# AI-Unicamp/GestureDiffusion

Hardware: AMD Instinct MI355X
Metric: denoised motion frames/sec (1000-step p_sample_loop, B=64, T=196, d=512) (higher is better)
Workload: dtype f32; 1 GPU; BASELINE config 2: MDM_Old (V1 encoder-only topology) J=263 d=512 ff=1024 L=8 H=4, 1000-step p_sample_loop, batch 64/GPU x 196 frames, random weights, in-kernel Philox noise; global_batch=64, frames=196, parallelism=dp1 (independent samples, end-of-loop gather), step=one denoising step (forward + fused sampler update) over the rank's batch

## Files before the change

gesturediffusion_amd/_lib.py:

```python
import ctypes as C
import os

_HERE = os.path.dirname(os.path.abspath(__file__))
LIB_PATH = os.environ.get("GDX_LIBGDX") or os.path.join(_HERE, "csrc", "libgdx.so")

GDX_ARCH_MDM_OLD, GDX_ARCH_MDM = 1, 2
GDX_COND, GDX_UNCOND, GDX_CFG = 0, 1, 2
GDX_SAMPLER_P, GDX_SAMPLER_DDIM = 0, 1
GDX_ROW_PAD = 256

EXPORTS = [
    "gdx_create", "gdx_destroy", "gdx_last_error", "gdx_set_weight", "gdx_weights_ready", "gdx_prepare",
    "gdx_set_condition", "gdx_forward", "gdx_set_keep_taps", "gdx_get_tap", "gdx_sampler_update", "gdx_q_sample",
    "gdx_randn", "gdx_sample_loop", "gdx_bench_ffn_gemm", "gdx_bench_gemm", "gdx_forward_flops", "gdx_profile_begin", "gdx_profile_end", "gdx_bench_attention",
    "gdx_linear_f16", "gdx_linear_f32", "gdx_bench_gemm_f16", "gdx_attention_f16", "gdx_attention_f32", "gdx_plms_update", "gdx_postprocess", "gdx_q_sample_t", "gdx_masked_l2", "gdx_set_graph_replay", "gdx_mfcc",
    "gdx_set_guards", "gdx_check_guards", "gdx_packed_bytes", "gdx_export_packed", "gdx_import_packed", "gdx_set_test_half_dtype",
    "gdx_set_test_gemmh_tile", "gdx_linear_half", "gdx_layernorm", "gdx_local_attention", "gdx_attention_half",
    "gdx_bpd_terms", "gdx_bpd_loop", "gdx_linear_full", "gdx_plms_step", "gdx_plms_loop",
    "gdx_dpm_step", "gdx_dpm_loop", "gdx_dpm_sde_step", "gdx_dpm_sde_loop",
    "gdx_set_guidance_interval", "gdx_forward_samples", "gdx_set_guidance_rescale", "gdx_cfg_rescale",
    "gdx_set_guidance_refresh", "gdx_cfg_delta",
    "gdx_transpose_in", "gdx_transpose_out", "gdx_small_linear", "gdx_gather_rows", "gdx_mfcc_project", "gdx_token0",
]
GDX_BPD_CHUNK = 4096
INT64_MIN, INT64_MAX = -2**63, 2**63 - 1


class GdxError(RuntimeError):
    pass


class Config(C.Structure):
    _fields_ = [(n, C.c_int32) for n in ("arch", "njoints", "latent_dim", "ff_size", "num_layers", "num_heads",
                                         "seed_poses", "mfcc_dim", "cl_head", "window", "compute_dtype")]


class UpdateArgs(C.Structure):
# ... 155 lines not shown
        "gdx_bench_attention": [i32, i32, i32, i32, i32, i32, C.POINTER(C.c_float), vp],
        "gdx_linear_f16": [vp, vp, vp, vp, vp, i32, i32, i32, i32, vp],
        "gdx_linear_f32": [vp, vp, vp, vp, vp, i32, i32, i32, i32, i32, i32, i32, vp],
        "gdx_linear_half": [vp, vp, vp, vp, i32, vp, i32, vp, vp, i32, i32, i32, i32, i32, i32, i32, i32, i32, i32,
                            C.POINTER(i32), vp],
        "gdx_linear_full": [vp, vp, vp, vp, i32, vp, i32, vp, i32, i32, i32, i32, i32, i32, i32, i32, i32, i32, i32,
                            C.POINTER(i32), vp],
        "gdx_layernorm": [vp, vp, vp, vp, vp, vp, i32, i32, i32, i32, i32, i32, vp],
        "gdx_local_attention": [vp, vp, vp, vp, vp, i32, i32, i32, i32, i32, i32, i32, C.POINTER(i32), vp],
        "gdx_transpose_in": [vp, vp, i32, i32, i32, i32, i32, i32, i32, vp],
        "gdx_transpose_out": [vp, vp, i32, i32, i32, i32, i32, vp],
        "gdx_small_linear": [vp, i32, vp, i32, vp, vp, i32, i32, i32, i32, i32, i32, vp],
        "gdx_gather_rows": [vp, vp, vp, i32, i32, i32, i32, vp],
        "gdx_mfcc_project": [vp, vp, i32, vp, vp, vp, i32, i32, i32, i32, i32, i32, i32, i32, vp],
        "gdx_token0": [vp, i32, vp, vp, vp, vp, i32, vp, vp, vp, i32, vp, i32, i32, i32, i32, i32, vp],
        "gdx_set_graph_replay": [vp, i32],
        "gdx_mfcc": [vp, i64, i32, i32, i32, i32, i32, i32, C.c_float, vp, vp, vp, vp, vp, vp, vp, vp, vp],
        "gdx_q_sample_t": [vp, vp, vp, vp, i32, i64, vp, vp],
        "gdx_masked_l2": [vp, vp, vp, vp, i32, i32, i32, vp],
        "gdx_postprocess": [vp, vp, vp, vp, vp, i32, i32, i32, vp],
        "gdx_plms_update": [C.POINTER(PlmsArgs), vp],
        "gdx_plms_step": [C.POINTER(PlmsStepArgs), vp],
        "gdx_plms_loop": [vp, C.POINTER(PlmsLoopArgs), vp],
        "gdx_dpm_step": [C.POINTER(DpmStepArgs), vp],
        "gdx_dpm_loop": [vp, C.POINTER(DpmLoopArgs), vp],
        "gdx_dpm_sde_step": [C.POINTER(DpmSdeStepArgs), vp],
        "gdx_dpm_sde_loop": [vp, C.POINTER(DpmSdeLoopArgs), vp],
        "gdx_attention_f16": [vp, vp, i32, i32, i32, i32, vp],
        "gdx_attention_half": [vp, i32, vp, i32, i32, i32, i32, i32, i32, i32, i32, C.POINTER(i32), vp],
        "gdx_attention_f32": [vp, vp, i32, i32, i32, i32, i32, vp],
# ... 32 lines not shown
```

gesturediffusion_amd/csrc/api.hip:

```cpp
#include "gdx_host.h"

#include <algorithm>
#include <cstdlib>
#include <cstring>
#include <string>
#include <vector>

namespace gdx {

static thread_local std::string g_err;

int fail(const std::string& m) {
    g_err = m;
    return -1;
}

}

using namespace gdx;

static constexpr size_t GUARD_BYTES = 64 * 1024;
static constexpr int GUARD_BYTE = 0xA5;

int gdx::dev_alloc(std::vector<void*>& pool, void** p, size_t bytes) {
// ... 267 lines not shown
    const int d = h->d;
    const bool res32 = !h->f16 || h->stream32;
    if (res32 ? linear(h, in, W, {.bias = W.bias, .R = resid.f, .ldr = d}, Act{h->tmp.f, nullptr}, d, N, d, s)
              : linear(h, in, W, {.bias = W.bias}, Act{nullptr, h->tmp.h}, d, N, d, s))
        return -1;
    for (const Act* o : {out, compact}) {
        if (!o) continue;
        const int cS = o == compact ? h->S : 0;
        if (res32) HIPCHK(HFN(h->bf16, launch_layernorm, h->tmp.f, nullptr, gamma, beta, o->f, o->h, N, d, cS, s));
        else HIPCHK(HFN(h->bf16, launch_layernorm_f16, h->tmp.h, resid.h, gamma, beta, o->h, o->f, N, d, cS, s));
    }
    return 0;
}

static int forward_core(gdx_model* h, const float* x, const float* temb, int tstride, const float* c2t, int mode,
                        float* x0_out, hipStream_t s, const int* state = nullptr, bool tm = false) {
    const int B = h->B, T = h->T, S = h->S, d = h->d, J = h->J;
    const int Beff = mode == GDX_CFG ? 2 * B : B;
    h->forward_samples += Beff;
    const float* seed_emb = mode == GDX_UNCOND ? h->seed_cat + (size_t)B * d : h->seed_cat;
    const int N = Beff * S;
    const Act xa{!h->f16 || h->stream32 || h->keep_taps ? h->xa.f : nullptr, h->xa.h};
    if (!tm && !h->f16) HIPCHK(launch_transpose_in(x, h->xt.f, Beff, B, J, T, h->in_x.kpad, s));
    if (!tm && h->f16) HIPCHK(HFN(h->bf16, launch_transpose_in_f16, x, h->xt.h, Beff, B, J, T, h->in_x.kpad16, s));
    if (h->cfg.arch == GDX_ARCH_MDM_OLD) {
        HIPCHK(HFN(h->bf16, launch_token0, temb, tstride, seed_emb, h->pe, h->xa.f, h->xa.h, nullptr, nullptr, nullptr, state, Beff, B, S, d, s));
        if (linear(h, h->xt, h->in_x, {.R = h->addend, .ldr = d, .rowmap = true}, xa, d, Beff * T, d, s)) return -1;
    } else {
        if (!c2t) return fail("forward_core: V2 needs the W_coa * temb rows");
        const float* c2s = mode == GDX_UNCOND ? h->c2_seed + (size_t)B * d : h->c2_seed;
        HIPCHK(HFN(h->bf16, launch_token0, temb, tstride, seed_emb, nullptr, h->xa.f, h->xa.h, c2t, c2s, h->c2, state, Beff, B, S, d, s));
        if (linear(h, h->xt, h->in_x, {.bias = h->in_x.bias}, h->emb, d, Beff * T, d, s)) return -1;
        const int dt = h->cfg.compute_dtype;
        const bool la16 = local_attention_half(dt, d, h->cfg.cl_head, h->cfg.window);
        const Act xseq = la16 ? Act{nullptr, h->xseq.h} : Act{h->xseq.f, nullptr};
        if (linear(h, h->emb, h->proj_pose, {.R = h->addend, .ldr = d, .V = h->c2, .ldv = d}, xseq, d, Beff * T, d, s)) return -1;
        HIPCHK(launch_local_attention_any(dt, h->xseq.f, h->xseq.h, h->rope_cos, h->rope_sin, la16 ? xa.f : h->xa.f, h->xa.h, Beff, T,
                                          d, h->cfg.cl_head, h->cfg.window, s));
    }
    auto tap = [&](int l) {
        if (h->keep_taps) HIPCHK(hipMemcpyAsync(h->taps[l], h->xa.f, sizeof(float) * (size_t)N * d, hipMemcpyDeviceToDevice, s));
// ... 186 lines not shown
    if (tables_live) return 0;
    h->tmap_host.assign(timestep_map, timestep_map + num_steps);
    HIPCHK(hipMemcpyAsync(h->tmap_dev, h->tmap_host.data(), sizeof(int64_t) * num_steps, hipMemcpyHostToDevice, s));
    float* scratch0 = table + (size_t)h->temb_table_rows * d;
    float* scratch1 = scratch0 + (size_t)h->temb_table_rows * d;
    if (time_embed(h, h->tmap_dev, num_steps, scratch0, scratch1, table, s)) return -1;
    if (h->cfg.arch == GDX_ARCH_MDM) {
        HIPCHK(launch_small_linear(table, d, h->proj_coa.w, h->proj_coa.kpad, nullptr, h->c2t_table, d, num_steps, d, d, 0, s));
        h->c2t_valid = true;
    }
    h->tables_valid = true;
    return 0;
}

static int denoise_step(gdx_model* h, const float* x, int idx, int mode, float* x0_out, hipStream_t s, const int* state = nullptr,
                        bool tm = false) {
    const size_t row = (size_t)idx * h->d;
    const int fm = mode == GDX_CFG_REFRESH ? GDX_CFG : mode == GDX_CFG_REUSE ? GDX_COND : mode;
    return forward_core(h, x, h->temb_table + row, 0, h->c2t_table ? h->c2t_table + row : nullptr, fm, x0_out, s, state, tm);
}

static const float* tape_slice(const float* tape, int k, int k_base, size_t rows, size_t per) {
    return tape ? tape + (ptrdiff_t)(k - k_base) * (ptrdiff_t)(rows * per) : nullptr;
}

static int denoise_guided(gdx_model* h, const CallSeq& q, const float* sc_in, const float* x, int idx, hipStream_t s,
                          const float** x0_uncond, const float** scale, bool second = false) {
    const int m = step_mode(h, q, idx, second);
    return denoise_step(h, x, idx, m, h->x0, s) || guided_operands(h, m, sc_in, s, x0_uncond, scale) ? -1 : 0;
}

extern "C" int gdx_bpd_loop(gdx_handle_t h, const gdx_bpd_loop_args_t* a, void* stream) {
    if (!h) return fail("gdx_bpd_loop: null handle");
    if (!a) return fail("gdx_bpd_loop: null argument");
// ... 192 lines not shown
    const bool refreshes = h->guide_every > 1 && any_guided;
    if (!((uintptr_t)a->noise_tape & 15) && !a->inpaint_mask && !a->n_dump && !h->graph_replay && !h->keep_taps && h->T % 4 == 0 &&
        !rescales && !refreshes) {
        static const bool mirror_always = [] { const char* e = getenv("GDX_TM_MIRROR"); return e && !strcmp(e, "always"); }();
        const int Beff = any_guided ? 2 * B : B;
        const int ldx = h->f16 ? h->in_x.kpad16 : h->in_x.kpad;
        HIPCHK(launch_transpose_in(a->x, h->xt.f, Beff, B, h->J, h->T, ldx, s));
        if (h->f16) HIPCHK(HFN(h->bf16, launch_transpose_in_f16, a->x, h->xt.h, Beff, B, h->J, h->T, ldx, s));
        gdx::UpdateTmDev u;
        memset(&u, 0, sizeof(u));
        u.kind = a->kind; u.B = B; u.J = h->J; u.T = h->T; u.ldx = ldx; u.ldo = h->ldo;
        u.coef = a->coef; u.xt = h->xt.f; u.x0t = h->x0t;
        u.const_noise = a->const_noise; u.seed = a->philox_seed; u.sample_offset = a->sample_offset;
        u.clip = a->clip_denoised;
        u.xt16 = h->xt.h; u.half_dtype = h->cfg.compute_dtype;
        int k = a->k_base;
        for (int idx = a->first_index; idx >= last_idx; --idx, ++k) {
            const int m = mode_at(idx);
            if (denoise_step(h, nullptr, idx, m, nullptr, s, nullptr, true)) return -1;
            u.scale = m == GDX_CFG ? a->scale : nullptr;
            u.mirror = any_guided && m != GDX_CFG && (mirror_always || (idx > last_idx && mode_at(idx - 1) == GDX_CFG));
            u.step_index = idx; u.rng_step = (uint32_t)(k + 1);
            u.out_pose = idx == last_idx ? a->x : nullptr;
            u.noise = tape_slice(a->noise_tape, k, a->k_base, tape_rows, per);
            if (gdx_sampler_update_tm_(u, stream)) return -1;
        }
        return 0;
    }
    const bool want_graph = h->graph_replay && !h->prof && !h->keep_taps && !a->n_dump && a->first_index - last_idx >= 8 && uniform && !refreshes;
    int idx = a->first_index, k = a->k_base;
    if (want_graph) {
        if (eager_step(idx, k)) return -1;
        --idx; ++k;
        bool ok = true;
// ... 150 lines not shown
```

gesturediffusion_amd/csrc/gdx_internal.h:

```cpp
#pragma once
#include <hip/hip_runtime.h>
#include <stdint.h>

#include "../../include/gdx.h"

#ifdef GDX_BF16
#define GDX_HNS_BEGIN namespace b16 {
#define GDX_HNS_NAME b16
#else
#define GDX_HNS_BEGIN inline namespace h16 {
#define GDX_HNS_NAME h16
#endif
#define GDX_HNS_END }

namespace gdx {

#ifdef GDX_BF16
typedef __bf16 half_t;
#else
typedef _Float16 half_t;
#endif

constexpr int ROW_PAD = GDX_ROW_PAD;

// ... 120 lines not shown
struct UpdateTmDev {
    int kind, B, J, T, ldx, ldo;
    const float* coef; int step_index;
    float* xt;
    const float* x0t;
    const float* scale;
    int const_noise;
    uint64_t seed, sample_offset;
    uint32_t rng_step;
    int clip;
    float* out_pose;
    void* xt16;
    int half_dtype;
    const float* noise;
    int mirror;
};

}

int gdx_sampler_update_state_(const gdx_update_args_t* a, const int* state, long noise_stride, void* stream);
int gdx_sampler_update_tm_(const gdx::UpdateTmDev& d, void* stream);
int gdx_bpd_xt_(const float* x0, const float* coef, int idx, int batch, long per_sample, uint64_t seed, uint64_t sample_offset,
                uint32_t step, float* z_out, float* xt_out, void* stream);
extern "C" int gdx_set_error_(const char* msg);
```

gesturediffusion_amd/csrc/misc.hip:

```cpp
#include "gdx_internal.h"
#include "gdx_device.h"

namespace gdx {
GDX_HNS_BEGIN

__device__ __forceinline__ float wave_sum(float v) {
#pragma unroll
    for (int o = 32; o > 0; o >>= 1) v += __shfl_xor(v, o);
    return v;
}

template <int VPL>
__global__ __launch_bounds__(256) void layernorm_vec_kernel(const float* __restrict__ x, const float* __restrict__ res,
                                                             const float* __restrict__ g,
                                                             const float* __restrict__ bta, float* __restrict__ out,
                                                             half_t* __restrict__ out16, int rows, int d,
                                                             int compact_S) {
    const int row = blockIdx.x * 4 + (threadIdx.x >> 6);
    const int lane = threadIdx.x & 63;
    if (row >= rows) return;
    long orow = row;
    if (compact_S > 0) {
        const int b = row / compact_S;
        if (row - b * compact_S == 0) return;
        orow = row - b - 1;
    }
    const f32x4* xp = reinterpret_cast<const f32x4*>(x + (long)row * d);
    const f32x4* rp = reinterpret_cast<const f32x4*>(res + (long)row * d);
    f32x4 v[VPL];
    float s = 0.0f;
#pragma unroll
    for (int i = 0; i < VPL; ++i) {
        v[i] = xp[lane + 64 * i];
        if (res) v[i] += rp[lane + 64 * i];
        s += (v[i][0] + v[i][1]) + (v[i][2] + v[i][3]);
    }
    const float mean = wave_sum(s) / (float)d;
    float q = 0.0f;
#pragma unroll
    for (int i = 0; i < VPL; ++i)
#pragma unroll
        for (int e = 0; e < 4; ++e) {
            const float c = v[i][e] - mean;
            q += c * c;
        }
    const float rstd = 1.0f / sqrtf(wave_sum(q) / (float)d + 1e-5f);
    f32x4* op = reinterpret_cast<f32x4*>(out + orow * d);
    f16x4* hp = reinterpret_cast<f16x4*>(out16 + orow * d);
    const f32x4* gp = reinterpret_cast<const f32x4*>(g);
    const f32x4* bp = reinterpret_cast<const f32x4*>(bta);
#pragma unroll
    for (int i = 0; i < VPL; ++i) {
        const f32x4 gg = gp[lane + 64 * i], bb = bp[lane + 64 * i];
        f32x4 r;
#pragma unroll
        for (int e = 0; e < 4; ++e) r[e] = (v[i][e] - mean) * rstd * gg[e] + bb[e];
        if (out) op[lane + 64 * i] = r;
        if (out16) hp[lane + 64 * i] = f16x4{(half_t)r[0], (half_t)r[1], (half_t)r[2], (half_t)r[3]};
    }
}

__global__ __launch_bounds__(256) void layernorm_gen_kernel(const float* __restrict__ x, const float* __restrict__ res,
                                                             const float* __restrict__ g,
                                                             const float* __restrict__ bta, float* __restrict__ out,
                                                             half_t* __restrict__ out16, int rows, int d,
                                                             int compact_S) {
    const int row = blockIdx.x * 4 + (threadIdx.x >> 6);
    const int lane = threadIdx.x & 63;
    if (row >= rows) return;
    long orow = row;
    if (compact_S > 0) {
        const int b = row / compact_S;
        if (row - b * compact_S == 0) return;
// ... 5 lines not shown
    for (int e = lane; e < d; e += 64) s += res ? xp[e] + rp[e] : xp[e];
    const float mean = wave_sum(s) / (float)d;
    float q = 0.0f;
    for (int e = lane; e < d; e += 64) {
        const float c = (res ? xp[e] + rp[e] : xp[e]) - mean;
        q += c * c;
    }
    const float rstd = 1.0f / sqrtf(wave_sum(q) / (float)d + 1e-5f);
    for (int e = lane; e < d; e += 64) {
        const float r = ((res ? xp[e] + rp[e] : xp[e]) - mean) * rstd * g[e] + bta[e];
        if (out) out[orow * d + e] = r;
        if (out16) out16[orow * d + e] = (half_t)r;
    }
}

hipError_t launch_layernorm(const float* x, const float* res, const float* gamma, const float* beta, float* out,
                            _Float16* out16_, int rows, int d, int compact_S, hipStream_t s) {
    half_t* out16 = reinterpret_cast<half_t*>(out16_);
    const dim3 grid((rows + 3) / 4), block(256);
    if (d == 512)
        hipLaunchKernelGGL(layernorm_vec_kernel<2>, grid, block, 0, s, x, res, gamma, beta, out, out16, rows, d, compact_S);
    else if (d == 1024)
        hipLaunchKernelGGL(layernorm_vec_kernel<4>, grid, block, 0, s, x, res, gamma, beta, out, out16, rows, d, compact_S);
    else if (d == 256)
        hipLaunchKernelGGL(layernorm_vec_kernel<1>, grid, block, 0, s, x, res, gamma, beta, out, out16, rows, d, compact_S);
    else
        hipLaunchKernelGGL(layernorm_gen_kernel, grid, block, 0, s, x, res, gamma, beta, out, out16, rows, d, compact_S);
    return hipGetLastError();
}

template <int NV>
__global__ __launch_bounds__(256) void layernorm_h_vec_kernel(const half_t* __restrict__ x, const half_t* __restrict__ res,
                                                               const float* __restrict__ g, const float* __restrict__ bta,
                                                               half_t* __restrict__ out16, float* __restrict__ out32,
                                                               int rows, int d, int compact_S) {
    const int row = blockIdx.x * 4 + (threadIdx.x >> 6);
    const int lane = threadIdx.x & 63;
    if (row >= rows) return;
    long orow = row;
    if (compact_S > 0) {
        const int b = row / compact_S;
        if (row - b * compact_S == 0) return;
// ... 750 lines not shown
```

gesturediffusion_amd/csrc/sampler.hip:

```cpp
#include <algorithm>
#include <string>

#include "gdx_internal.h"
#include "gdx_device.h"
#include "../../include/gdx.h"

#pragma clang fp contract(off)

namespace gdx {


struct Philox {
    static constexpr uint32_t M0 = 0xD2511F53u, M1 = 0xCD9E8D57u, W0 = 0x9E3779B9u, W1 = 0xBB67AE85u;
    __device__ static void run(uint32_t c[4], uint32_t k0, uint32_t k1) {
#pragma unroll
        for (int r = 0; r < 10; ++r) {
            const uint32_t hi0 = __umulhi(M0, c[0]), lo0 = M0 * c[0];
            const uint32_t hi1 = __umulhi(M1, c[2]), lo1 = M1 * c[2];
            const uint32_t n0 = hi1 ^ c[1] ^ k0, n2 = hi0 ^ c[3] ^ k1;
            c[0] = n0; c[1] = lo1; c[2] = n2; c[3] = lo0;
            k0 += W0; k1 += W1;
        }
    }
};
// ... 169 lines not shown
    const f32x4 x = load4<VEC>(a.s.x, g.e0, g.nval);
    const f32x4 x0 = pred_xstart4<VEC>(a.s, g);
    const f32x4 z = noise ? load4<VEC>(noise, a.const_noise ? 4L * g.grp : g.e0, g.nval)
                          : philox_normal4(a.seed, a.const_noise ? 0ull : a.sample_offset + (uint64_t)g.b, rng_step, g.grp);
    const bool cond = a.grad != nullptr;
    const f32x4 grad = cond ? load4<VEC>(a.grad, g.e0, g.nval) : f32x4{0.f, 0.f, 0.f, 0.f};
    const float s1m = cond && a.kind != GDX_SAMPLER_P ? a.gcoef[idx] : 0.0f;
    f32x4 r;
#pragma unroll
    for (int i = 0; i < 4; ++i) r[i] = update_value(a.kind, c, x[i], x0[i], z[i], cond, grad[i], s1m);
    store4<VEC>(a.s.out, g.e0, g.nval, r);
    if (a.s.pred) store4<VEC>(a.s.pred, g.e0, g.nval, x0);
}

__global__ __launch_bounds__(256) void update_tm_kernel(const UpdateTmDev a) {
    const int jq_n = (a.J + 3) / 4, tq_n = a.T / 4;
    const long gid = (long)blockIdx.x * 256 + threadIdx.x;
    if (gid >= (long)a.B * tq_n * jq_n) return;
    const int jq = gid % jq_n;
    const long bt = gid / jq_n;
    const int tq = bt % tq_n, b = bt / tq_n;
    const int j0 = 4 * jq, t0 = 4 * tq;
    const float* c = a.coef + (long)a.step_index * 8;
    const long row0 = (long)b * a.T + t0;
    const long urow = (long)a.B * a.T;
    const bool both = a.scale || a.mirror;
    f32x4 x[4], x0[4];
#pragma unroll
    for (int tt = 0; tt < 4; ++tt) {
        x[tt] = *reinterpret_cast<const f32x4*>(a.xt + (row0 + tt) * a.ldx + j0);
        x0[tt] = *reinterpret_cast<const f32x4*>(a.x0t + (row0 + tt) * a.ldo + j0);
    }
    if (a.scale) {
        const float sc = a.scale[b];
#pragma unroll
        for (int tt = 0; tt < 4; ++tt) {
            const f32x4 u = *reinterpret_cast<const f32x4*>(a.x0t + (urow + row0 + tt) * a.ldo + j0);
#pragma unroll
            for (int jj = 0; jj < 4; ++jj) x0[tt][jj] = cfg_blend(x0[tt][jj], u[jj], sc);
        }
    }
    if (a.clip) {
#pragma unroll
        for (int tt = 0; tt < 4; ++tt)
#pragma unroll
            for (int jj = 0; jj < 4; ++jj) x0[tt][jj] = clamp1(x0[tt][jj]);
    }
    const uint64_t sample = a.const_noise ? 0ull : a.sample_offset + (uint64_t)b;
    f32x4 r[4];
#pragma unroll
    for (int jj = 0; jj < 4; ++jj) {
        const int j = j0 + jj;
        if (j < a.J) {
            const f32x4 z = a.noise ? *reinterpret_cast<const f32x4*>(a.noise + ((long)(a.const_noise ? 0 : b) * a.J + j) * a.T + t0)
                                    : philox_normal4(a.seed, sample, a.rng_step, (uint32_t)(j * tq_n + tq));
#pragma unroll
            for (int tt = 0; tt < 4; ++tt) r[tt][jj] = update_value(a.kind, c, x[tt][jj], x0[tt][jj], z[tt]);
        } else {
#pragma unroll
            for (int tt = 0; tt < 4; ++tt) r[tt][jj] = 0.0f;
        }
    }
#pragma unroll
    for (int tt = 0; tt < 4; ++tt) {
        *reinterpret_cast<f32x4*>(a.xt + (row0 + tt) * a.ldx + j0) = r[tt];
        if (both) *reinterpret_cast<f32x4*>(a.xt + (urow + row0 + tt) * a.ldx + j0) = r[tt];
    }
    if (a.xt16) {
        typedef _Float16 h4 __attribute__((ext_vector_type(4)));
        typedef __bf16 b4 __attribute__((ext_vector_type(4)));
#pragma unroll
        for (int tt = 0; tt < 4; ++tt) {
            const long o0 = (row0 + tt) * a.ldx + j0, o1 = o0 + urow * a.ldx;
            if (a.half_dtype == GDX_DTYPE_BF16) {
                const b4 v = b4{(__bf16)r[tt][0], (__bf16)r[tt][1], (__bf16)r[tt][2], (__bf16)r[tt][3]};
                *reinterpret_cast<b4*>((__bf16*)a.xt16 + o0) = v;
                if (both) *reinterpret_cast<b4*>((__bf16*)a.xt16 + o1) = v;
            } else {
                const h4 v = h4{(_Float16)r[tt][0], (_Float16)r[tt][1], (_Float16)r[tt][2], (_Float16)r[tt][3]};
                *reinterpret_cast<h4*>((_Float16*)a.xt16 + o0) = v;
                if (both) *reinterpret_cast<h4*>((_Float16*)a.xt16 + o1) = v;
            }
        }
    }
    if (a.out_pose) {
#pragma unroll
        for (int jj = 0; jj < 4; ++jj)
            if (j0 + jj < a.J)
                *reinterpret_cast<f32x4*>(a.out_pose + ((long)b * a.J + j0 + jj) * a.T + t0) = f32x4{r[0][jj], r[1][jj], r[2][jj], r[3][jj]};
    }
}

__global__ void q_sample_kernel(const float* __restrict__ xs, const float* __restrict__ nz, const float* coef,
                                int idx, const int64_t* __restrict__ t, long per_sample, long n, float* __restrict__ out) {
    const long i = (long)blockIdx.x * blockDim.x + threadIdx.x;
    if (i >= n) return;
    const long row = t ? (long)t[i / per_sample] : (long)idx;
    const float a = coef[row * 8 + 5], b = coef[row * 8 + 6];
    out[i] = q_sample_value(a, b, xs[i], nz[i]);
}

__global__ void plms_kernel(int kind, const float* __restrict__ coef, const int64_t* __restrict__ t, int step_index,
                            const float* __restrict__ x, const float* __restrict__ x0, const float* __restrict__ e0,
                            const float* __restrict__ e1, const float* __restrict__ e2, const float* __restrict__ e3,
                            float* __restrict__ out, long per_sample, long total) {
// ... 437 lines not shown
    if (const char* m = hist_check()) return refuse(who, m);
    s = step_src(a, a->*pred);
    if (a->batch == 0 || s.per_sample == 0) return 1;
    grid = dim3((unsigned)((s.groups + 255) / 256), (unsigned)a->batch);
    return 0;
}

static int sampler_update_impl(const gdx_update_args_t* a, const int* state, long noise_stride, void* stream);

int gdx_sampler_update_tm_(const gdx::UpdateTmDev& d, void* stream) {
    using namespace gdx;
    const int jpad = (d.J + 3) / 4 * 4;
    if (!d.coef || !d.xt || !d.x0t || d.T % 4 || d.ldx % 4 || d.ldo % 4 || d.ldx < jpad || d.ldo < jpad)
        return gdx_set_error_("gdx_sampler_update_tm_: bad argument");
    if (d.noise && ((uintptr_t)d.noise & 15)) return gdx_set_error_("gdx_sampler_update_tm_: noise tape not 16-byte aligned");
    const long total = (long)d.B * (d.T / 4) * (jpad / 4);
    if (total == 0) return 0;
    hipLaunchKernelGGL(update_tm_kernel, dim3((total + 255) / 256), dim3(256), 0, (hipStream_t)stream, d);
    return launch_status("gdx_sampler_update_tm_: launch failed");
}

extern "C" int gdx_sampler_update(const gdx_update_args_t* a, void* stream) {
    return sampler_update_impl(a, nullptr, 0, stream);
}

int gdx_sampler_update_state_(const gdx_update_args_t* a, const int* state, long noise_stride, void* stream) {
    return sampler_update_impl(a, state, noise_stride, stream);
}

static int sampler_update_impl(const gdx_update_args_t* a, const int* state, long noise_stride, void* stream) {
    using namespace gdx;
// ... 264 lines not shown
```

gesturediffusion_amd/csrc/testapi.hip:

```cpp
#include "gdx_host.h"

#include <cstdio>
#include <cstdlib>

using namespace gdx;

static bool t_bf16 = false;
static int t_gemmh_mb = -1, t_gemmh_nbw = -1;

namespace {

struct Scratch {
    const std::string who;
    const hipStream_t s;
    const bool bf;
    std::vector<void*> pool;
    Scratch(const char* who, hipStream_t s, bool bf = false) : who(who), s(s), bf(bf) {}
    ~Scratch() {
        (void)hipStreamSynchronize(s);
        free_pool(pool);
    }
    template <class T>
    int alloc(T** p, size_t bytes) { return dev_alloc(pool, (void**)p, bytes); }
    int to_half(_Float16** h, const float* src, int64_t n) {
// ... 348 lines not shown
        return fail("gdx_token0: c2t, c2_seed and c2 go together");
    if (enc_rows < (long)(B - 1) * S + 1) return fail("gdx_token0: enc_rows below the stored rows");
    if (c2 && c2_rows < B) return fail("gdx_token0: c2_rows below B");
    hipStream_t s = (hipStream_t)stream;
    const int64_t n_enc = (int64_t)enc_rows * d, n_c2 = (int64_t)c2_rows * d;
    float *e32 = nullptr, *o2 = nullptr;
    _Float16* e16 = nullptr;
    Scratch sc("gdx_token0", s, dtype == GDX_DTYPE_BF16);
    if (sc.stage(&e32, enc, n_enc) || (enc16 && sc.to_half(&e16, enc16, n_enc)) || (c2 && sc.stage(&o2, c2, n_c2))) return -1;
    const hipError_t e = HFN(sc.bf, launch_token0, temb, tstride, seed_emb, pe0, e32, e16, c2t, c2_seed, o2, state, B, Bsrc, S, d, s);
    if (e != hipSuccess) return fail(std::string("launch_token0: ") + hipGetErrorString(e));
    if (sc.unstage(e32, enc, n_enc) || (c2 && sc.unstage(o2, c2, n_c2))) return -1;
    return enc16 ? sc.widen(e16, enc16, n_enc) : 0;
}

extern "C" int gdx_attention_f16(const float* qkv, float* ctx, int32_t B, int32_t S, int32_t H, int32_t d, void* stream) {
    if (!qkv || !ctx || B <= 0 || S <= 0 || H <= 0 || d <= 0 || d % H || !HFN(t_bf16, attentionh_supported, S, H, d))
        return fail("gdx_attention_f16: bad argument / unsupported shape (head_dim " GDX_HEAD_DIMS ")");
    hipStream_t s = (hipStream_t)stream;
    const size_t rows = (size_t)B * S;
    _Float16 *q16 = nullptr, *c16 = nullptr;
    Scratch sc("gdx_attention_f16", s, t_bf16);
    if (sc.to_half(&q16, qkv, (int64_t)rows * 3 * d) || sc.to_half(&c16, nullptr, (int64_t)rows * d)) return -1;
    const hipError_t e = HFN(sc.bf, launch_attentionh, q16, c16, B, S, H, d, (long)rows, s);
    if (e != hipSuccess) return fail(std::string("launch_attentionh: ") + hipGetErrorString(e));
    return sc.widen(c16, ctx, (int64_t)rows * d);
}

extern "C" int gdx_attention_half(const float* qkv, int32_t qkv_rows, float* ctx, int32_t ctx_rows, int32_t B, int32_t S,
                                  int32_t H, int32_t d, int32_t dtype, int32_t kernel, int32_t grid, int32_t* launched,
// ... 119 lines not shown
```

include/gdx.h:

```cpp
#ifndef GDX_H
#define GDX_H

#include <stdint.h>

#ifdef __cplusplus
extern "C" {
#endif

typedef struct gdx_model* gdx_handle_t;

#define GDX_ROW_PAD 256

enum { GDX_ARCH_MDM_OLD = 1,
       GDX_ARCH_MDM = 2 };

enum { GDX_COND = 0,
       GDX_UNCOND = 1,
       GDX_CFG = 2 };

enum { GDX_DTYPE_F32 = 0,
       GDX_DTYPE_F16 = 1,
       GDX_DTYPE_BF16 = 2 };

enum { GDX_SAMPLER_P = 0,
// ... 345 lines not shown
                        int32_t B, int32_t T, int32_t d, int32_t heads, int32_t window, int32_t dtype, int32_t* kernel,
                        void* stream);
int gdx_transpose_in(const float* x, float* xt, int32_t xt_rows, int32_t B, int32_t Bsrc, int32_t J, int32_t T, int32_t ldx,
                     int32_t dtype, void* stream);
int gdx_transpose_out(const float* yt, float* y, int32_t y_rows, int32_t B, int32_t J, int32_t T, int32_t ldy, void* stream);
int gdx_small_linear(const float* A, int32_t lda, const float* W, int32_t ldw, const float* bias, float* out, int32_t out_rows,
                     int32_t ldo, int32_t M, int32_t N, int32_t K, int32_t act, void* stream);
int gdx_gather_rows(const float* table, const int64_t* idx, float* out, int32_t out_rows, int32_t M, int32_t d,
                    int32_t max_rows, void* stream);
int gdx_mfcc_project(const float* mfcc, const float* W, int32_t ldw, const float* bias, const float* pe, float* out,
                     int32_t out_rows, int32_t B, int32_t Bsrc, int32_t C, int32_t T, int32_t d, int32_t rps, int32_t off,
                     void* stream);
int gdx_token0(const float* temb, int32_t tstride, const float* seed_emb, const float* pe0, float* enc, float* enc16,
               int32_t enc_rows, const float* c2t, const float* c2_seed, float* c2, int32_t c2_rows, const int32_t* state,
               int32_t B, int32_t Bsrc, int32_t S, int32_t d, int32_t dtype, void* stream);
int gdx_attention_f16(const float* qkv, float* ctx, int32_t B, int32_t S, int32_t H, int32_t d, void* stream);
int gdx_attention_half(const float* qkv, int32_t qkv_rows, float* ctx, int32_t ctx_rows, int32_t B, int32_t S, int32_t H,
                       int32_t d, int32_t dtype, int32_t kernel, int32_t grid, int32_t* launched, void* stream);
int gdx_set_test_half_dtype(int32_t dtype);
int gdx_set_test_gemmh_tile(int32_t mb, int32_t nbw);
int gdx_attention_f32(const float* qkv, float* ctx, int32_t B, int32_t S, int32_t H, int32_t d, int32_t version,
                      void* stream);
int gdx_linear_f32(const float* A, const float* W, const float* bias, const float* R, float* C, int32_t M, int32_t N,
                   int32_t K, int32_t epi, int32_t tile_mb, int32_t tile_nbw, int32_t tile_bk, void* stream);
int gdx_linear_full(const float* A, const float* W, const float* bias, const float* R, int32_t ldr, const float* V,
                    int32_t ldv, float* C, int32_t c_rows, int32_t M, int32_t N, int32_t K, int32_t T, int32_t rowmap,
                    int32_t gelu, int32_t kernel, int32_t tile_mb, int32_t tile_nbw, int32_t tile_bk, int32_t* launched,
                    void* stream);
int gdx_bench_gemm_f16(int32_t M, int32_t N, int32_t K, int32_t gelu, int32_t iters, float* avg_us,
                       void* stream);
// ... 7 lines not shown
```

Before: 3101 frames/s.

## Fold token0 into sampler update, persistent layernorm, per-joint update threads

Folds the conditioning-token write for the next step into the fused sampler update kernel, so one launch per denoising step goes away for the MDM_Old topology. Rewrites the vector layernorm as a persistent grid-stride kernel capped at a few workgroups per CU, with gamma/beta held in registers and the next row prefetched. Rewrites the tm update kernel to one thread per joint handling four frames, which gives up the 4x4 vectorised f32x4 loads and stores for scalar strided accesses. Also adds a test entry point for the tm update.

Result: no change. 3126 frames/s (median of 6 runs) (+0.8%).

```diff
diff --git a/gesturediffusion_amd/_lib.py b/gesturediffusion_amd/_lib.py
--- a/gesturediffusion_amd/_lib.py
+++ b/gesturediffusion_amd/_lib.py
@@ -21,6 +21,7 @@
     "gdx_set_guidance_interval", "gdx_forward_samples", "gdx_set_guidance_rescale", "gdx_cfg_rescale",
     "gdx_set_guidance_refresh", "gdx_cfg_delta",
     "gdx_transpose_in", "gdx_transpose_out", "gdx_small_linear", "gdx_gather_rows", "gdx_mfcc_project", "gdx_token0",
+    "gdx_update_tm",
 ]
 GDX_BPD_CHUNK = 4096
 INT64_MIN, INT64_MAX = -2**63, 2**63 - 1
@@ -206,6 +207,8 @@
         "gdx_gather_rows": [vp, vp, vp, i32, i32, i32, i32, vp],
         "gdx_mfcc_project": [vp, vp, i32, vp, vp, vp, i32, i32, i32, i32, i32, i32, i32, i32, vp],
         "gdx_token0": [vp, i32, vp, vp, vp, vp, i32, vp, vp, vp, i32, vp, i32, i32, i32, i32, i32, vp],
+        "gdx_update_tm": [i32, i32, i32, i32, i32, i32, vp, i32, vp, vp, i32, vp, vp, i32, vp, i32, u64, u64, u32, i32, vp, i32,
+                          vp],
         "gdx_set_graph_replay": [vp, i32],
         "gdx_mfcc": [vp, i64, i32, i32, i32, i32, i32, i32, C.c_float, vp, vp, vp, vp, vp, vp, vp, vp, vp],
         "gdx_q_sample_t": [vp, vp, vp, vp, i32, i64, vp, vp],
diff --git a/gesturediffusion_amd/csrc/api.hip b/gesturediffusion_amd/csrc/api.hip
--- a/gesturediffusion_amd/csrc/api.hip
+++ b/gesturediffusion_amd/csrc/api.hip
@@ -305,7 +305,7 @@
 }
 
 static int forward_core(gdx_model* h, const float* x, const float* temb, int tstride, const float* c2t, int mode,
-                        float* x0_out, hipStream_t s, const int* state = nullptr, bool tm = false) {
+                        float* x0_out, hipStream_t s, const int* state = nullptr, bool tm = false, bool tok0_done = false) {
     const int B = h->B, T = h->T, S = h->S, d = h->d, J = h->J;
     const int Beff = mode == GDX_CFG ? 2 * B : B;
     h->forward_samples += Beff;
@@ -315,7 +315,8 @@
     if (!tm && !h->f16) HIPCHK(launch_transpose_in(x, h->xt.f, Beff, B, J, T, h->in_x.kpad, s));
     if (!tm && h->f16) HIPCHK(HFN(h->bf16, launch_transpose_in_f16, x, h->xt.h, Beff, B, J, T, h->in_x.kpad16, s));
     if (h->cfg.arch == GDX_ARCH_MDM_OLD) {
-        HIPCHK(HFN(h->bf16, launch_token0, temb, tstride, seed_emb, h->pe, h->xa.f, h->xa.h, nullptr, nullptr, nullptr, state, Beff, B, S, d, s));
+        if (!tok0_done)
+            HIPCHK(HFN(h->bf16, launch_token0, temb, tstride, seed_emb, h->pe, h->xa.f, h->xa.h, nullptr, nullptr, nullptr, state, Beff, B, S, d, s));
         if (linear(h, h->xt, h->in_x, {.R = h->addend, .ldr = d, .rowmap = true}, xa, d, Beff * T, d, s)) return -1;
     } else {
         if (!c2t) return fail("forward_core: V2 needs the W_coa * temb rows");
@@ -532,10 +533,10 @@
 }
 
 static int denoise_step(gdx_model* h, const float* x, int idx, int mode, float* x0_out, hipStream_t s, const int* state = nullptr,
-                        bool tm = false) {
+                        bool tm = false, bool tok0_done = false) {
     const size_t row = (size_t)idx * h->d;
     const int fm = mode == GDX_CFG_REFRESH ? GDX_CFG : mode == GDX_CFG_REUSE ? GDX_COND : mode;
-    return forward_core(h, x, h->temb_table + row, 0, h->c2t_table ? h->c2t_table + row : nullptr, fm, x0_out, s, state, tm);
+    return forward_core(h, x, h->temb_table + row, 0, h->c2t_table ? h->c2t_table + row : nullptr, fm, x0_out, s, state, tm, tok0_done);
 }
 
 static const float* tape_slice(const float* tape, int k, int k_base, size_t rows, size_t per) {
@@ -758,10 +759,19 @@
         u.const_noise = a->const_noise; u.seed = a->philox_seed; u.sample_offset = a->sample_offset;
         u.clip = a->clip_denoised;
         u.xt16 = h->xt.h; u.half_dtype = h->cfg.compute_dtype;
+        const bool fold_tok0 = h->cfg.arch == GDX_ARCH_MDM_OLD;
+        u.tok_S = h->S; u.tok_d = h->d; u.tok_pe0 = h->pe; u.tok_enc = h->xa.f; u.tok_enc16 = h->xa.h;
         int k = a->k_base;
         for (int idx = a->first_index; idx >= last_idx; --idx, ++k) {
             const int m = mode_at(idx);
-            if (denoise_step(h, nullptr, idx, m, nullptr, s, nullptr, true)) return -1;
+            if (denoise_step(h, nullptr, idx, m, nullptr, s, nullptr, true, fold_tok0 && idx != a->first_index)) return -1;
+            u.tok_n = 0;
+            if (fold_tok0 && idx > last_idx) {
+                const int mn = mode_at(idx - 1);
+                u.tok_n = (mn == GDX_CFG ? 2 * B : B) * h->d;
+                u.tok_temb = h->temb_table + (size_t)(idx - 1) * h->d;
+                u.tok_seed = mn == GDX_UNCOND ? h->seed_cat + (size_t)B * h->d : h->seed_cat;
+            }
             u.scale = m == GDX_CFG ? a->scale : nullptr;
             u.mirror = any_guided && m != GDX_CFG && (mirror_always || (idx > last_idx && mode_at(idx - 1) == GDX_CFG));
             u.step_index = idx; u.rng_step = (uint32_t)(k + 1);
diff --git a/gesturediffusion_amd/csrc/gdx_internal.h b/gesturediffusion_amd/csrc/gdx_internal.h
--- a/gesturediffusion_amd/csrc/gdx_internal.h
+++ b/gesturediffusion_amd/csrc/gdx_internal.h
@@ -158,6 +158,10 @@
     int half_dtype;
     const float* noise;
     int mirror;
+    int tok_n, tok_S, tok_d;
+    const float *tok_temb, *tok_seed, *tok_pe0;
+    float* tok_enc;
+    void* tok_enc16;
 };
 
 }
diff --git a/gesturediffusion_amd/csrc/misc.hip b/gesturediffusion_amd/csrc/misc.hip
--- a/gesturediffusion_amd/csrc/misc.hip
+++ b/gesturediffusion_amd/csrc/misc.hip
@@ -2,6 +2,7 @@
 #include "gdx_device.h"
 
 namespace gdx {
+int gemm2_num_cus();
 GDX_HNS_BEGIN
 
 __device__ __forceinline__ float wave_sum(float v) {
@@ -10,53 +11,71 @@
     return v;
 }
 
+constexpr int LN_WG_PER_CU = 4;
+constexpr int LN_WAVES = 4;
 template <int VPL>
-__global__ __launch_bounds__(256) void layernorm_vec_kernel(const float* __restrict__ x, const float* __restrict__ res,
+__global__ __launch_bounds__(64 * LN_WAVES) void layernorm_vec_kernel(const float* __restrict__ x, const float* __restrict__ res,
                                                              const float* __restrict__ g,
                                                              const float* __restrict__ bta, float* __restrict__ out,
                                                              half_t* __restrict__ out16, int rows, int d,
                                                              int compact_S) {
-    const int row = blockIdx.x * 4 + (threadIdx.x >> 6);
     const int lane = threadIdx.x & 63;
+    const int nwaves = gridDim.x * LN_WAVES;
+    int row = blockIdx.x * LN_WAVES + (threadIdx.x >> 6);
     if (row >= rows) return;
-    long orow = row;
-    if (compact_S > 0) {
-        const int b = row / compact_S;
-        if (row - b * compact_S == 0) return;
-        orow = row - b - 1;
-    }
-    const f32x4* xp = reinterpret_cast<const f32x4*>(x + (long)row * d);
-    const f32x4* rp = reinterpret_cast<const f32x4*>(res + (long)row * d);
-    f32x4 v[VPL];
-    float s = 0.0f;
+    f32x4 v[VPL], gg[VPL], bb[VPL];
+    auto load_row = [&](f32x4 (&t)[VPL], int r) {
+        const f32x4* xp = reinterpret_cast<const f32x4*>(x + (long)r * d);
+        const f32x4* rp = reinterpret_cast<const f32x4*>(res + (long)r * d);
+#pragma unroll
+        for (int i = 0; i < VPL; ++i) {
+            t[i] = xp[lane + 64 * i];
+            if (res) t[i] += rp[lane + 64 * i];
+        }
+    };
+    load_row(v, row);
 #pragma unroll
     for (int i = 0; i < VPL; ++i) {
-        v[i] = xp[lane + 64 * i];
-        if (res) v[i] += rp[lane + 64 * i];
-        s += (v[i][0] + v[i][1]) + (v[i][2] + v[i][3]);
-    }
-    const float mean = wave_sum(s) / (float)d;
-    float q = 0.0f;
-#pragma unroll
-    for (int i = 0; i < VPL; ++i)
-#pragma unroll
-        for (int e = 0; e < 4; ++e) {
-            const float c = v[i][e] - mean;
-            q += c * c;
-        }
-    const float rstd = 1.0f / sqrtf(wave_sum(q) / (float)d + 1e-5f);
-    f32x4* op = reinterpret_cast<f32x4*>(out + orow * d);
-    f16x4* hp = reinterpret_cast<f16x4*>(out16 + orow * d);
-    const f32x4* gp = reinterpret_cast<const f32x4*>(g);
-    const f32x4* bp = reinterpret_cast<const f32x4*>(bta);
-#pragma unroll
-    for (int i = 0; i < VPL; ++i) {
-        const f32x4 gg = gp[lane + 64 * i], bb = bp[lane + 64 * i];
-        f32x4 r;
-#pragma unroll
-        for (int e = 0; e < 4; ++e) r[e] = (v[i][e] - mean) * rstd * gg[e] + bb[e];
-        if (out) op[lane + 64 * i] = r;
-        if (out16) hp[lane + 64 * i] = f16x4{(half_t)r[0], (half_t)r[1], (half_t)r[2], (half_t)r[3]};
+        gg[i] = reinterpret_cast<const f32x4*>(g)[lane + 64 * i];
+        bb[i] = reinterpret_cast<const f32x4*>(bta)[lane + 64 * i];
+    }
+    for (; row < rows; row += nwaves) {
+        f32x4 nx[VPL];
+        load_row(nx, row + nwaves < rows ? row + nwaves : row);
+        float s = 0.0f;
+#pragma unroll
+        for (int i = 0; i < VPL; ++i) s += (v[i][0] + v[i][1]) + (v[i][2] + v[i][3]);
+        const float mean = wave_sum(s) / (float)d;
+        float q = 0.0f;
+#pragma unroll
+        for (int i = 0; i < VPL; ++i)
+#pragma unroll
+            for (int e = 0; e < 4; ++e) {
+                const float c = v[i][e] - mean;
+                q += c * c;
+            }
+        const float rstd = 1.0f / sqrtf(wave_sum(q) / (float)d + 1e-5f);
+        long orow = row;
+        bool keep = true;
+        if (compact_S > 0) {
+            const int b = row / compact_S;
+            keep = row - b * compact_S != 0;
+            orow = row - b - 1;
+        }
+        if (keep) {
+            f32x4* op = reinterpret_cast<f32x4*>(out + orow * d);
+            f16x4* hp = reinterpret_cast<f16x4*>(out16 + orow * d);
+#pragma unroll
+            for (int i = 0; i < VPL; ++i) {
+                f32x4 r;
+#pragma unroll
+                for (int e = 0; e < 4; ++e) r[e] = (v[i][e] - mean) * rstd * gg[i][e] + bb[i][e];
+                if (out) op[lane + 64 * i] = r;
+                if (out16) hp[lane + 64 * i] = f16x4{(half_t)r[0], (half_t)r[1], (half_t)r[2], (half_t)r[3]};
+            }
+        }
+#pragma unroll
+        for (int i = 0; i < VPL; ++i) v[i] = nx[i];
     }
 }
 
@@ -92,18 +111,26 @@
     }
 }
 
+template <int VPL>
+static void launch_ln_vec(const float* x, const float* res, const float* gamma, const float* beta, float* out, half_t* out16,
+                          int rows, int d, int compact_S, hipStream_t s) {
+    const int wgs = (rows + LN_WAVES - 1) / LN_WAVES, resident = gemm2_num_cus() * LN_WG_PER_CU;
+    hipLaunchKernelGGL(layernorm_vec_kernel<VPL>, dim3(wgs < resident ? wgs : resident), dim3(64 * LN_WAVES), 0, s, x, res,
+                       gamma, beta, out, out16, rows, d, compact_S);
+}
+
 hipError_t launch_layernorm(const float* x, const float* res, const float* gamma, const float* beta, float* out,
                             _Float16* out16_, int rows, int d, int compact_S, hipStream_t s) {
     half_t* out16 = reinterpret_cast<half_t*>(out16_);
-    const dim3 grid((rows + 3) / 4), block(256);
     if (d == 512)
-        hipLaunchKernelGGL(layernorm_vec_kernel<2>, grid, block, 0, s, x, res, gamma, beta, out, out16, rows, d, compact_S);
+        launch_ln_vec<2>(x, res, gamma, beta, out, out16, rows, d, compact_S, s);
     else if (d == 1024)
-        hipLaunchKernelGGL(layernorm_vec_kernel<4>, grid, block, 0, s, x, res, gamma, beta, out, out16, rows, d, compact_S);
+        launch_ln_vec<4>(x, res, gamma, beta, out, out16, rows, d, compact_S, s);
     else if (d == 256)
-        hipLaunchKernelGGL(layernorm_vec_kernel<1>, grid, block, 0, s, x, res, gamma, beta, out, out16, rows, d, compact_S);
+        launch_ln_vec<1>(x, res, gamma, beta, out, out16, rows, d, compact_S, s);
     else
-        hipLaunchKernelGGL(layernorm_gen_kernel, grid, block, 0, s, x, res, gamma, beta, out, out16, rows, d, compact_S);
+        hipLaunchKernelGGL(layernorm_gen_kernel, dim3((rows + 3) / 4), dim3(256), 0, s, x, res, gamma, beta, out, out16, rows,
+                           d, compact_S);
     return hipGetLastError();
 }
 
diff --git a/gesturediffusion_amd/csrc/sampler.hip b/gesturediffusion_amd/csrc/sampler.hip
--- a/gesturediffusion_amd/csrc/sampler.hip
+++ b/gesturediffusion_amd/csrc/sampler.hip
@@ -207,81 +207,76 @@
 }
 
 __global__ __launch_bounds__(256) void update_tm_kernel(const UpdateTmDev a) {
-    const int jq_n = (a.J + 3) / 4, tq_n = a.T / 4;
+    const int jp = (a.J + 3) / 4 * 4, tq_n = a.T / 4;
     const long gid = (long)blockIdx.x * 256 + threadIdx.x;
-    if (gid >= (long)a.B * tq_n * jq_n) return;
-    const int jq = gid % jq_n;
-    const long bt = gid / jq_n;
+    const long groups = (long)a.B * tq_n * jp;
+    if (gid >= groups) {
+        const long i = gid - groups;
+        if (i < a.tok_n) {
+            const int b = i / a.tok_d, n = i % a.tok_d;
+            float v = a.tok_temb[n] + a.tok_seed[i];
+            if (a.tok_pe0) v += a.tok_pe0[n];
+            const long o = (long)b * a.tok_S * a.tok_d + n;
+            a.tok_enc[o] = v;
+            if (a.tok_enc16) {
+                if (a.half_dtype == GDX_DTYPE_BF16) ((__bf16*)a.tok_enc16)[o] = (__bf16)v;
+                else ((_Float16*)a.tok_enc16)[o] = (_Float16)v;
+            }
+        }
+        return;
+    }
+    const int j = gid % jp;
+    const long bt = gid / jp;
     const int tq = bt % tq_n, b = bt / tq_n;
-    const int j0 = 4 * jq, t0 = 4 * tq;
+    const int t0 = 4 * tq;
     const float* c = a.coef + (long)a.step_index * 8;
     const long row0 = (long)b * a.T + t0;
     const long urow = (long)a.B * a.T;
     const bool both = a.scale || a.mirror;
-    f32x4 x[4], x0[4];
+    float* xp = a.xt + row0 * a.ldx + j;
+    f32x4 r = f32x4{0.0f, 0.0f, 0.0f, 0.0f};
+    if (j < a.J) {
+        const float* x0p = a.x0t + row0 * a.ldo + j;
+        f32x4 x, x0;
+#pragma unroll
+        for (int tt = 0; tt < 4; ++tt) {
+            x[tt] = xp[(long)tt * a.ldx];
+            x0[tt] = x0p[(long)tt * a.ldo];
+        }
+        if (a.scale) {
+            const float sc = a.scale[b];
+#pragma unroll
+            for (int tt = 0; tt < 4; ++tt) x0[tt] = cfg_blend(x0[tt], x0p[(urow + tt) * a.ldo], sc);
+        }
+        if (a.clip) {
+#pragma unroll
+            for (int tt = 0; tt < 4; ++tt) x0[tt] = clamp1(x0[tt]);
+        }
+        const uint64_t sample = a.const_noise ? 0ull : a.sample_offset + (uint64_t)b;
+        const f32x4 z = a.noise ? *reinterpret_cast<const f32x4*>(a.noise + ((long)(a.const_noise ? 0 : b) * a.J + j) * a.T + t0)
+                                : philox_normal4(a.seed, sample, a.rng_step, (uint32_t)(j * tq_n + tq));
+#pragma unroll
+        for (int tt = 0; tt < 4; ++tt) r[tt] = update_value(a.kind, c, x[tt], x0[tt], z[tt]);
+    }
 #pragma unroll
     for (int tt = 0; tt < 4; ++tt) {
-        x[tt] = *reinterpret_cast<const f32x4*>(a.xt + (row0 + tt) * a.ldx + j0);
-        x0[tt] = *reinterpret_cast<const f32x4*>(a.x0t + (row0 + tt) * a.ldo + j0);
-    }
-    if (a.scale) {
-        const float sc = a.scale[b];
+        xp[(long)tt * a.ldx] = r[tt];
+        if (both) xp[(urow + tt) * a.ldx] = r[tt];
+    }
+    if (a.xt16) {
 #pragma unroll
         for (int tt = 0; tt < 4; ++tt) {
-            const f32x4 u = *reinterpret_cast<const f32x4*>(a.x0t + (urow + row0 + tt) * a.ldo + j0);
-#pragma unroll
-            for (int jj = 0; jj < 4; ++jj) x0[tt][jj] = cfg_blend(x0[tt][jj], u[jj], sc);
-        }
-    }
-    if (a.clip) {
-#pragma unroll
-        for (int tt = 0; tt < 4; ++tt)
-#pragma unroll
-            for (int jj = 0; jj < 4; ++jj) x0[tt][jj] = clamp1(x0[tt][jj]);
-    }
-    const uint64_t sample = a.const_noise ? 0ull : a.sample_offset + (uint64_t)b;
-    f32x4 r[4];
-#pragma unroll
-    for (int jj = 0; jj < 4; ++jj) {
-        const int j = j0 + jj;
-        if (j < a.J) {
-            const f32x4 z = a.noise ? *reinterpret_cast<const f32x4*>(a.noise + ((long)(a.const_noise ? 0 : b) * a.J + j) * a.T + t0)
-                                    : philox_normal4(a.seed, sample, a.rng_step, (uint32_t)(j * tq_n + tq));
-#pragma unroll
-            for (int tt = 0; tt < 4; ++tt) r[tt][jj] = update_value(a.kind, c, x[tt][jj], x0[tt][jj], z[tt]);
-        } else {
-#pragma unroll
-            for (int tt = 0; tt < 4; ++tt) r[tt][jj] = 0.0f;
-        }
-    }
-#pragma unroll
-    for (int tt = 0; tt < 4; ++tt) {
-        *reinterpret_cast<f32x4*>(a.xt + (row0 + tt) * a.ldx + j0) = r[tt];
-        if (both) *reinterpret_cast<f32x4*>(a.xt + (urow + row0 + tt) * a.ldx + j0) = r[tt];
-    }
-    if (a.xt16) {
-        typedef _Float16 h4 __attribute__((ext_vector_type(4)));
-        typedef __bf16 b4 __attribute__((ext_vector_type(4)));
-#pragma unroll
-        for (int tt = 0; tt < 4; ++tt) {
-            const long o0 = (row0 + tt) * a.ldx + j0, o1 = o0 + urow * a.ldx;
+            const long o0 = (row0 + tt) * a.ldx + j, o1 = o0 + urow * a.ldx;
             if (a.half_dtype == GDX_DTYPE_BF16) {
-                const b4 v = b4{(__bf16)r[tt][0], (__bf16)r[tt][1], (__bf16)r[tt][2], (__bf16)r[tt][3]};
-                *reinterpret_cast<b4*>((__bf16*)a.xt16 + o0) = v;
-                if (both) *reinterpret_cast<b4*>((__bf16*)a.xt16 + o1) = v;
+                ((__bf16*)a.xt16)[o0] = (__bf16)r[tt];
+                if (both) ((__bf16*)a.xt16)[o1] = (__bf16)r[tt];
             } else {
-                const h4 v = h4{(_Float16)r[tt][0], (_Float16)r[tt][1], (_Float16)r[tt][2], (_Float16)r[tt][3]};
-                *reinterpret_cast<h4*>((_Float16*)a.xt16 + o0) = v;
-                if (both) *reinterpret_cast<h4*>((_Float16*)a.xt16 + o1) = v;
+                ((_Float16*)a.xt16)[o0] = (_Float16)r[tt];
+                if (both) ((_Float16*)a.xt16)[o1] = (_Float16)r[tt];
             }
         }
     }
-    if (a.out_pose) {
-#pragma unroll
-        for (int jj = 0; jj < 4; ++jj)
-            if (j0 + jj < a.J)
-                *reinterpret_cast<f32x4*>(a.out_pose + ((long)b * a.J + j0 + jj) * a.T + t0) = f32x4{r[0][jj], r[1][jj], r[2][jj], r[3][jj]};
-    }
+    if (a.out_pose && j < a.J) *reinterpret_cast<f32x4*>(a.out_pose + ((long)b * a.J + j) * a.T + t0) = r;
 }
 
 __global__ void q_sample_kernel(const float* __restrict__ xs, const float* __restrict__ nz, const float* coef,
@@ -749,7 +744,9 @@
     if (!d.coef || !d.xt || !d.x0t || d.T % 4 || d.ldx % 4 || d.ldo % 4 || d.ldx < jpad || d.ldo < jpad)
         return gdx_set_error_("gdx_sampler_update_tm_: bad argument");
     if (d.noise && ((uintptr_t)d.noise & 15)) return gdx_set_error_("gdx_sampler_update_tm_: noise tape not 16-byte aligned");
-    const long total = (long)d.B * (d.T / 4) * (jpad / 4);
+    if (d.tok_n < 0 || (d.tok_n > 0 && (!d.tok_temb || !d.tok_seed || !d.tok_enc || d.tok_d <= 0 || d.tok_S <= 0)))
+        return gdx_set_error_("gdx_sampler_update_tm_: bad conditioning-token argument");
+    const long total = (long)d.B * (d.T / 4) * jpad + d.tok_n;
     if (total == 0) return 0;
     hipLaunchKernelGGL(update_tm_kernel, dim3((total + 255) / 256), dim3(256), 0, (hipStream_t)stream, d);
     return launch_status("gdx_sampler_update_tm_: launch failed");
diff --git a/gesturediffusion_amd/csrc/testapi.hip b/gesturediffusion_amd/csrc/testapi.hip
--- a/gesturediffusion_amd/csrc/testapi.hip
+++ b/gesturediffusion_amd/csrc/testapi.hip
@@ -386,6 +386,30 @@
     return enc16 ? sc.widen(e16, enc16, n_enc) : 0;
 }
 
+extern "C" int gdx_update_tm(int32_t kind, int32_t B, int32_t J, int32_t T, int32_t ldx, int32_t ldo, const float* coef,
+                             int32_t step_index, float* xt, float* xt16, int32_t xt_rows, const float* x0t, const float* scale,
+                             int32_t mirror, const float* noise, int32_t const_noise, uint64_t philox_seed, uint64_t sample_offset,
+                             uint32_t rng_step, int32_t clip_denoised, float* out_pose, int32_t dtype, void* stream) {
+    if (!coef || !xt || !x0t || B <= 0 || J <= 0 || T <= 0 || step_index < 0 || (kind != GDX_SAMPLER_P && kind != GDX_SAMPLER_DDIM))
+        return fail("gdx_update_tm: bad argument");
+    if (!dtype_known(dtype)) return fail("gdx_update_tm: unknown dtype");
+    if (xt16 && dtype == GDX_DTYPE_F32) return fail("gdx_update_tm: GDX_DTYPE_F32 takes no xt16");
+    if (scale && mirror) return fail("gdx_update_tm: mirror belongs to an unguided step");
+    if (xt_rows < (long)(scale || mirror ? 2 : 1) * B * T) return fail("gdx_update_tm: xt_rows below the stored rows");
+    hipStream_t s = (hipStream_t)stream;
+    const int64_t n = (int64_t)xt_rows * ldx;
+    _Float16* h16 = nullptr;
+    Scratch sc("gdx_update_tm", s, dtype == GDX_DTYPE_BF16);
+    if (xt16 && sc.to_half(&h16, xt16, n)) return -1;
+    gdx::UpdateTmDev u{};
+    u.kind = kind; u.B = B; u.J = J; u.T = T; u.ldx = ldx; u.ldo = ldo;
+    u.coef = coef; u.step_index = step_index; u.xt = xt; u.x0t = x0t; u.scale = scale; u.mirror = mirror;
+    u.const_noise = const_noise; u.seed = philox_seed; u.sample_offset = sample_offset; u.rng_step = rng_step;
+    u.clip = clip_denoised; u.out_pose = out_pose; u.xt16 = h16; u.half_dtype = dtype; u.noise = noise;
+    if (gdx_sampler_update_tm_(u, stream)) return -1;
+    return xt16 ? sc.widen(h16, xt16, n) : 0;
+}
+
 extern "C" int gdx_attention_f16(const float* qkv, float* ctx, int32_t B, int32_t S, int32_t H, int32_t d, void* stream) {
     if (!qkv || !ctx || B <= 0 || S <= 0 || H <= 0 || d <= 0 || d % H || !HFN(t_bf16, attentionh_supported, S, H, d))
         return fail("gdx_attention_f16: bad argument / unsupported shape (head_dim " GDX_HEAD_DIMS ")");
diff --git a/include/gdx.h b/include/gdx.h
--- a/include/gdx.h
+++ b/include/gdx.h
@@ -383,6 +383,10 @@
 int gdx_token0(const float* temb, int32_t tstride, const float* seed_emb, const float* pe0, float* enc, float* enc16,
                int32_t enc_rows, const float* c2t, const float* c2_seed, float* c2, int32_t c2_rows, const int32_t* state,
                int32_t B, int32_t Bsrc, int32_t S, int32_t d, int32_t dtype, void* stream);
+int gdx_update_tm(int32_t kind, int32_t B, int32_t J, int32_t T, int32_t ldx, int32_t ldo, const float* coef,
+                  int32_t step_index, float* xt, float* xt16, int32_t xt_rows, const float* x0t, const float* scale,
+                  int32_t mirror, const float* noise, int32_t const_noise, uint64_t philox_seed, uint64_t sample_offset,
+                  uint32_t rng_step, int32_t clip_denoised, float* out_pose, int32_t dtype, void* stream);
 int gdx_attention_f16(const float* qkv, float* ctx, int32_t B, int32_t S, int32_t H, int32_t d, void* stream);
 int gdx_attention_half(const float* qkv, int32_t qkv_rows, float* ctx, int32_t ctx_rows, int32_t B, int32_t S, int32_t H,
                        int32_t d, int32_t dtype, int32_t kernel, int32_t grid, int32_t* launched, void* stream);
```
